# UtkarshMishra04/bioimitation-gym

Hardware: AMD Instinct MI355X
Metric: env steps/sec (whole node), MuscleWalkingImitation2D-v0 @ 4096 envs/GPU (higher is better)
Workload: dtype f64

## Files before the change

### bioimitation-gym_amd/csrc/bioim_step.hip

```cpp
#include <hip/hip_runtime.h>

#include <math.h>
#include <stdint.h>
#include <stdio.h>
#include <string.h>

#include <string>
#include <type_traits>
#include <memory>
#include <vector>

#include "bioim.h"
#include "bioim_device.h"
#include "topologies.h"

#define DEV __device__ __forceinline__
#define BIOIM_EPB 16
#define BIOIM_STRUCT_FLAGS (BIOIM_ENV_MUSCLE | BIOIM_ENV_HAS_TZ | BIOIM_ENV_REWARD_FEET | BIOIM_ENV_DONE_CROSS | BIOIM_ENV_PD)

#ifndef BIOIM_CHECK
#define BIOIM_CHECK 0
#endif
DEV size_t bioim_chk(size_t i, size_t n, int line) {
    if (i >= n) {
// ... 542 lines not shown
    static constexpr int U = ((MF + 3 * (NSLOT > 0 ? NSLOT : 1) + 1) / 2) * 2;
    static constexpr int LOC = U;
    static constexpr int SL = LOC + 24 * (NB + 1);
    static constexpr int TZ = MPL * T::G * T::MAXSPAN;
    static constexpr int TAUN = TZ + 1;
    static constexpr int TAU = U;
    static constexpr int CJ = TAU + TAUN;
    static constexpr int OBS = U;
    static constexpr int REP = OBS + OBSMAX;
    static constexpr int U1 = 24 * (NB + 1) + 6 * (ND + 1), U2 = TAUN + NS * CJN;
    static constexpr int U3 = OBSMAX + 6 * (T::NOS + 1);
    static constexpr int USZ = U1 > U2 ? (U1 > U3 ? U1 : U3) : (U2 > U3 ? U2 : U3);
    static constexpr int SIZE0 = ((U + USZ + 1) / 2) * 2;
    static constexpr int SIZE = (BIOIM_ENV_MOD >= 0 && T::PLANAR) ? SIZE0 + ((BIOIM_ENV_MOD - SIZE0 % 32) + 32) % 32 : SIZE0;
};

#ifndef BIOIM_REALIZE_CACHE
#define BIOIM_REALIZE_CACHE 1
#endif
#ifndef BIOIM_REALIZE_CACHE_SPATIAL
#define BIOIM_REALIZE_CACHE_SPATIAL 1
#endif
#ifndef BIOIM_REALIZE_CACHE_TORQUE
#define BIOIM_REALIZE_CACHE_TORQUE 1
#endif
#ifndef BIOIM_CACHE_PREFETCH_SPATIAL
#define BIOIM_CACHE_PREFETCH_SPATIAL 0
#endif
template <class T> struct CacheLay {
    static constexpr bool ON = BIOIM_REALIZE_CACHE &&
                               (T::NM > 0 ? (T::PLANAR || BIOIM_REALIZE_CACHE_SPATIAL) : BIOIM_REALIZE_CACHE_TORQUE);
    static constexpr bool PREFETCH = T::PLANAR || BIOIM_CACHE_PREFETCH_SPATIAL;
    static constexpr int ND = T::ND > 0 ? T::ND : 1, NP = ND * (ND + 1) / 2;
    static constexpr int SYS = NP + ND;
    static constexpr int MUS = SYS;
    static constexpr int H = MUS + 3 * T::NM;
    static constexpr int DIM = ON ? H + 1 : 0;
    static constexpr int PF = (SYS + T::G - 1) / T::G;
};

constexpr int PERT_SLOT = 5;

DEV void wave_sync() {
    __builtin_amdgcn_fence(__ATOMIC_RELEASE, "wavefront");
    __builtin_amdgcn_wave_barrier();
    __builtin_amdgcn_fence(__ATOMIC_ACQUIRE, "wavefront");
}
DEV void wave_sync_lanes() { wave_sync(); }

#ifdef BIOIM_STAMPS
#define STAMP(i)                                                                      \
    do {                                                                              \
        __builtin_amdgcn_sched_barrier(0);                                            \
        unsigned long long t_ = __builtin_amdgcn_s_memtime();                         \
        __builtin_amdgcn_s_waitcnt(0xC07F);                                           \
        if (blockIdx.x == 0 && threadIdx.x == 0) g_stamps[i] += t_ - stamp_prev;      \
        stamp_prev = t_;                                                              \
        __builtin_amdgcn_sched_barrier(0);                                            \
    } while (0)
#define STAMP_DECL unsigned long long stamp_prev = __builtin_amdgcn_s_memtime();
#else
#define STAMP(i) do {} while (0)
#define STAMP_DECL
#endif

template <int I> DEV constexpr int tri(int k, int l) { return k * (k + 1) / 2 + l; }

template <class T, typename Real>
DEV void publish_coords(const DModel<Real> &M, const SModel<T, Real> &SM, Real *lds, int lane, Real qd, Real ud) {
    using LY = Lay<T, Real>;
    if (lane < T::ND) {
        const int c = SM.dof_coord[lane];
        lds[LY::QF + c] = qd;
        lds[LY::UF + c] = ud;
    }
    if (lane == 0) {
        sfor<0, T::NC>([&](auto cI) {
            constexpr int c = decltype(cI)::value;
            if constexpr (T::coord_dof[c] < 0) { lds[LY::QF + c] = M.coord_default[c]; lds[LY::UF + c] = 0; }
        });
    }
}

template <class T, typename Real>
DEV void kin_local(const SModel<T, Real> &SM, Real *lds, int c) {
    using LY = Lay<T, Real>;
    using PL = Planar<T>;
    constexpr unsigned ZR = PL::ZR, ZW = PL::ZW, ZV = PL::ZV;
    constexpr unsigned USED = TopoInfo<T>::axes_used();
    const SBody<Real> &b = SM.body[c];
    Real RFM[9] = {1, 0, 0, 0, 1, 0, 0, 0, 1};
    Real wrel[3] = {0, 0, 0}, arel[3] = {0, 0, 0}, pFM[3] = {0, 0, 0}, pd[3] = {0, 0, 0}, pdd[3] = {0, 0, 0};
    Real col[6][3];
    int cd[6];
    sfor<0, 6>([&](auto aI) {
        constexpr int ax = decltype(aI)::value;
        cd[ax] = -1;
        if constexpr (((USED >> ax) & 1u) != 0) {
            int kind = -1, cc = -1, dof = -1, js = -1;
            int cb = c;
            if constexpr (!T::PLANAR) asm volatile("" : "+v"(cb));
            sfor<0, T::NB>([&](auto bI) {
                constexpr int bb = decltype(bI)::value;
                constexpr int k = T::axis_kind[bb * 6 + ax], co = T::axis_coord[bb * 6 + ax];
                constexpr int dc = co >= 0 ? T::coord_dof[co] : -1, jsl = TopoInfo<T>::jslot(bb, ax);
                kind = cb == bb ? k : kind;
                cc = cb == bb ? co : cc;
                dof = cb == bb ? dc : dof;
                js = cb == bb ? jsl : js;
            });
            const int cs = cc >= 0 ? cc : 0;
            Real qc = lds[LY::QF + cs], uc = lds[LY::UF + cs];
            qc = cc >= 0 ? qc : Real(0);
            uc = cc >= 0 ? uc : Real(0);
            constexpr unsigned KM = TopoInfo<T>::axis_kinds(ax);
            const Real fa = b.fa[ax], fb = b.fb[ax];
            Real f = 0, f1 = 0, f2 = 0;
            if constexpr ((KM & (1u << (BIOIM_FN_LINEAR + 1))) != 0) {
                if (kind == BIOIM_FN_LINEAR) { f = fa * qc + fb; f1 = fa; }
            }
            if constexpr ((KM & (1u << (BIOIM_FN_CONST + 1))) != 0) {
                if (kind == BIOIM_FN_CONST) f = fb;
            }
            if constexpr ((KM & (1u << (BIOIM_FN_SPLINE + 1))) != 0) {
                const int jj = js >= 0 ? js : 0;
                if constexpr (T::PLANAR) {
                    const bool sp = kind == BIOIM_FN_SPLINE;
                    const Real sf = lds[LY::MF + 3 * jj], sf1 = lds[LY::MF + 3 * jj + 1], sf2 = lds[LY::MF + 3 * jj + 2];
                    f = sp ? sf : f; f1 = sp ? sf1 : f1; f2 = sp ? sf2 : f2;
                } else if (kind == BIOIM_FN_SPLINE) {
                    f = lds[LY::MF + 3 * jj]; f1 = lds[LY::MF + 3 * jj + 1]; f2 = lds[LY::MF + 3 * jj + 2];
                }
            }
            cd[ax] = dof;
            Real a[3] = {b.axis[ax][0], b.axis[ax][1], b.axis[ax][2]};
            if constexpr (ax < 3) {
                PL::ang(a);
                Real ucol[3], cr[3];
                mv3m<ZR, ZW>(RFM, a, ucol);
                Real thd = f1 * uc;
                cross3m<ZW, ZW>(wrel, ucol, cr);
#pragma unroll
                for (int i = 0; i < 3; ++i) {
                    arel[i] += ucol[i] * (f2 * uc * uc) + cr[i] * thd;
                    wrel[i] += ucol[i] * thd;
                    col[ax][i] = ucol[i] * f1;
                }
                PL::ang(arel); PL::ang(wrel); PL::ang(col[ax]);
                Real Rk[9];
                if constexpr (T::PLANAR) {
                    Real sn, cn;
                    sincos_rt(f, sn, cn);
                    Rk[0] = cn; Rk[1] = -sn * a[2]; Rk[3] = sn * a[2]; Rk[4] = cn;
                    PL::rot(Rk);
                } else {
                    axis_rot(a, f, Rk);
                }
                mm3m<ZR, ZR>(RFM, Rk, RFM);
            } else {
#pragma unroll
                for (int i = 0; i < 3; ++i) {
                    pFM[i] += a[i] * f; pd[i] += a[i] * (f1 * uc); pdd[i] += a[i] * (f2 * uc * uc);
                    col[ax][i] = a[i] * f1;
                }
                PL::lin(pd); PL::lin(pdd); PL::lin(col[ax]);
            }
        }
    });
    Real Rpf[9], Rmb[9];
#pragma unroll
    for (int i = 0; i < 9; ++i) { Rpf[i] = b.R_pf[i]; Rmb[i] = b.R_mb[i]; }
    PL::rot(Rpf); PL::rot(Rmb);
    Real dF[3], T9[9], RPB[9], pm[3], pPB[3];
    mv3m<ZR, 0>(RFM, b.p_mb, dF);
    mm3m<ZR, ZR>(Rpf, RFM, T9);
    mm3m<ZR, ZR>(T9, Rmb, RPB);
#pragma unroll
    for (int i = 0; i < 3; ++i) pm[i] = pFM[i] + dF[i];
    mv3m<ZR, 0>(Rpf, pm, pPB);
    Real *lc = lds + LY::LOC + 24 * c;
#pragma unroll
    for (int i = 0; i < 9; ++i) lc[i] = RPB[i];
#pragma unroll
    for (int i = 0; i < 3; ++i) lc[9 + i] = pPB[i] + b.p_pf[i];
    Real t1[3], t2[3], t3[3], o[3];
    mv3m<ZR, ZW>(Rpf, wrel, o);
#pragma unroll
    for (int i = 0; i < 3; ++i) lc[12 + i] = o[i];
    cross3m<ZW, 0>(wrel, dF, t1);
#pragma unroll
    for (int i = 0; i < 3; ++i) t2[i] = pd[i] + t1[i];
    mv3m<ZR, ZV>(Rpf, t2, o);
#pragma unroll
    for (int i = 0; i < 3; ++i) lc[15 + i] = o[i];
    mv3m<ZR, ZW>(Rpf, arel, o);
#pragma unroll
    for (int i = 0; i < 3; ++i) lc[18 + i] = o[i];
    cross3m<ZW, 0>(arel, dF, t2);
    cross3m<ZW, ZV>(wrel, t1, t3);
#pragma unroll
    for (int i = 0; i < 3; ++i) t2[i] = pdd[i] + t2[i] + t3[i];
    mv3m<ZR, ZV>(Rpf, t2, o);
#pragma unroll
    for (int i = 0; i < 3; ++i) lc[21 + i] = o[i];
    Real pM[3];
    mv3m<ZR, 0>(Rpf, pFM, pM);
#pragma unroll
    for (int i = 0; i < 3; ++i) pM[i] += b.p_pf[i];
    sfor<0, 6>([&](auto aI) {
        constexpr int ax = decltype(aI)::value;
        if constexpr (((USED >> ax) & 1u) != 0) {
            if (T::PLANAR || cd[ax] >= 0) {
                Real *sl = lds + LY::SL + 6 * (cd[ax] >= 0 ? cd[ax] : LY::ND);
                Real v[3];
                if constexpr (ax < 3) {
                    mv3m<ZR, ZW>(Rpf, col[ax], v);
                    Real lin[3];
                    cross3m<0, ZW>(pM, v, lin);
#pragma unroll
                    for (int i = 0; i < 3; ++i) {
                        if (!((ZW >> i) & 1u)) sl[i] += v[i];
                        if (!((ZV >> i) & 1u)) sl[3 + i] += lin[i];
                    }
                } else {
                    mv3m<ZR, ZV>(Rpf, col[ax], v);
#pragma unroll
                    for (int i = 0; i < 3; ++i)
                        if (!((ZV >> i) & 1u)) sl[3 + i] += v[i];
                }
            }
        }
    });
}

template <typename Real> struct Frame {
    Real R[9], o[3], w[3], vO[3], al[3], aO[3];
};

template <class T, typename Real> DEV void compose(Frame<Real> &F, const Real *lc) {
    using PL = Planar<T>;
    constexpr unsigned ZR = PL::ZR, ZW = PL::ZW, ZV = PL::ZV;
    Real R[9], oB[3], w[3], wrg[3], vrel[3], vO[3], al[3], t[3], t2[3], t3[3];
    mm3m<ZR, ZR>(F.R, lc, R);
    mv3m<ZR, 0>(F.R, lc + 9, t);
#pragma unroll
    for (int i = 0; i < 3; ++i) oB[i] = F.o[i] + t[i];
    mv3m<ZR, ZW>(F.R, lc + 12, wrg);
#pragma unroll
    for (int i = 0; i < 3; ++i) w[i] = F.w[i] + wrg[i];
    mv3m<ZR, ZV>(F.R, lc + 15, vrel);
    cross3m<ZW, 0>(wrg, oB, t);
#pragma unroll
    for (int i = 0; i < 3; ++i) vO[i] = F.vO[i] + vrel[i] - t[i];
    mv3m<ZR, ZW>(F.R, lc + 18, t);
    cross3m<ZW, ZW>(F.w, wrg, t2);
#pragma unroll
    for (int i = 0; i < 3; ++i) al[i] = F.al[i] + t2[i] + t[i];
    Real vpt[3], aB[3], aa[3];
    cross3m<ZW, 0>(F.w, oB, t);
#pragma unroll
    for (int i = 0; i < 3; ++i) vpt[i] = F.vO[i] + t[i];
    cross3m<ZW, 0>(F.al, oB, t);
    cross3m<ZW, ZV>(F.w, vpt, t2);
    cross3m<ZW, ZV>(F.w, vrel, t3);
    mv3m<ZR, ZV>(F.R, lc + 21, aa);
#pragma unroll
    for (int i = 0; i < 3; ++i) aB[i] = F.aO[i] + t[i] + t2[i] + Real(2) * t3[i] + aa[i];
    Real vB[3];
    cross3m<ZW, 0>(w, oB, t);
#pragma unroll
    for (int i = 0; i < 3; ++i) vB[i] = vO[i] + t[i];
    cross3m<ZW, 0>(al, oB, t);
    cross3m<ZW, ZV>(w, vB, t2);
#pragma unroll
    for (int i = 0; i < 9; ++i) F.R[i] = R[i];
#pragma unroll
    for (int i = 0; i < 3; ++i) {
        F.aO[i] = aB[i] - t[i] - t2[i];
        F.o[i] = oB[i]; F.w[i] = w[i]; F.vO[i] = vO[i]; F.al[i] = al[i];
    }
    PL::rot(F.R); PL::ang(F.w); PL::lin(F.vO); PL::ang(F.al); PL::lin(F.aO);
}

#ifndef BIOIM_GROUND_ONCE
#define BIOIM_GROUND_ONCE 3
#endif
template <class T, typename Real> DEV constexpr bool ground_loc_free() {
    using LY = Lay<T, Real>;
    return LY::LOC + 24 * T::NB >= LY::TAU + LY::TAUN && LY::LOC + 24 * T::NB >= LY::CJ + LY::NS * LY::CJN;
}
template <class T, typename Real> DEV void kin_ground_loc(Real *lds) {
    Real *lc = lds + Lay<T, Real>::LOC + 24 * T::NB;
#pragma unroll
    for (int i = 0; i < 24; ++i) lc[i] = (i < 9 && (i % 4) == 0) ? Real(1) : Real(0);
}
template <class T, typename Real> DEV void kin_ground_const(Real *lds) {
    using LY = Lay<T, Real>;
    Real *kb = lds + LY::KB + 18 * T::NB, *ab = lds + LY::AL + 6 * T::NB;
#pragma unroll
    for (int i = 0; i < 18; ++i) kb[i] = (i < 9 && (i % 4) == 0) ? Real(1) : Real(0);
#pragma unroll
    for (int i = 0; i < 6; ++i) ab[i] = 0;
}
template <class T, typename Real, bool ONCE = false> DEV void kin_ground(Real *lds, Real x0) {
    if constexpr (!ONCE || !ground_loc_free<T, Real>()) kin_ground_loc<T, Real>(lds);
    if constexpr (!ONCE) kin_ground_const<T, Real>(lds);
    lds[Lay<T, Real>::KB + 18 * T::NB + 9] = -x0;
}

template <class T, typename Real>
DEV void kin_chain(const SModel<T, Real> &SM, Real *lds, int c, Real x0) {
    using LY = Lay<T, Real>;
    Frame<Real> F;
#pragma unroll
    for (int i = 0; i < 9; ++i) F.R[i] = (i % 4) == 0 ? Real(1) : Real(0);
#pragma unroll
    for (int i = 0; i < 3; ++i) { F.o[i] = i == 0 ? -x0 : Real(0); F.w[i] = 0; F.vO[i] = 0; F.al[i] = 0; F.aO[i] = 0; }
    sfor<0, TopoInfo<T>::depth()>([&](auto lI) {
        constexpr int lvl = decltype(lI)::value;
        const Real *src = lds + LY::LOC + 24 * SM.chain[c][lvl];
        Real lc[24];
#pragma unroll
        for (int i = 0; i < 24; ++i) lc[i] = src[i];
        Planar<T>::loc(lc);
        compose<T, Real>(F, lc);
    });
    Real *kb = lds + LY::KB + 18 * c, *ab = lds + LY::AL + 6 * c;
#pragma unroll
    for (int i = 0; i < 9; ++i) kb[i] = F.R[i];
#pragma unroll
    for (int i = 0; i < 3; ++i) {
        kb[9 + i] = F.o[i]; kb[12 + i] = F.w[i]; kb[15 + i] = F.vO[i];
        ab[i] = F.al[i]; ab[3 + i] = F.aO[i];
    }
}

template <bool BFK, class T, typename Real>
DEV void fn_slots(const SModel<T, Real> &SM, Real *lds, int lane) {
    using LY = Lay<T, Real>;
    if constexpr (LY::NSLOT > 0) {
        sfor<0, (LY::NSLOT + T::G - 1) / T::G>([&](auto pI) {
            const int f = lane + decltype(pI)::value * T::G;
            if (f < LY::NSLOT) {
                Real v, d1, d2;
                fn_eval_bf<BFK, T, Real>(SM, SM.mf_fn[f], lds[LY::QF + SM.mf_coord[f]], v, d1, d2);
                lds[LY::MF + 3 * f] = v;
                lds[LY::MF + 3 * f + 1] = d1;
                lds[LY::MF + 3 * f + 2] = d2;
            }
        });
        wave_sync();
    }
}

template <class T, typename Real>
DEV void kin_column(const SModel<T, Real> &SM, Real *lds, int d) {
    using LY = Lay<T, Real>;
    using PL = Planar<T>;
    constexpr unsigned ZR = PL::ZR, ZW = PL::ZW, ZV = PL::ZV;
    const Real *kp = lds + LY::KB + 18 * SM.body[SM.dof_cb[d]].pslot;
    const Real *sl = lds + LY::SL + 6 * d;
    Real K[12], sc[6];
#pragma unroll
    for (int i = 0; i < 12; ++i) K[i] = kp[i];
#pragma unroll
    for (int i = 0; i < 6; ++i) sc[i] = sl[i];
    PL::rot(K); PL::col(sc);
    Real Sa[3], Sl[3], t[3];
    mv3m<ZR, ZW>(K, sc, Sa);
    mv3m<ZR, ZV>(K, sc + 3, Sl);
    cross3m<ZW, 0>(Sa, K + 9, t);
    Real *S = lds + LY::S + 6 * d;
#pragma unroll
    for (int i = 0; i < 3; ++i) { S[i] = Sa[i]; S[3 + i] = Sl[i] - t[i]; }
}

template <class T, typename Real>
DEV void body_inertia(const SModel<T, Real> &SM, const DModel<Real> &M, Real *lds, int c) {
    using LY = Lay<T, Real>;
    using PL = Planar<T>;
    constexpr unsigned ZR = PL::ZR, ZW = PL::ZW, ZV = PL::ZV;
    const SBody<Real> &b = SM.body[c];
    const Real *kb = lds + LY::KB + 18 * c, *ab = lds + LY::AL + 6 * c;
    Real K[18], A[6];
#pragma unroll
    for (int i = 0; i < 18; ++i) K[i] = kb[i];
#pragma unroll
    for (int i = 0; i < 6; ++i) A[i] = ab[i];
    PL::frame(K); PL::acc(A);
    const Real *R = K, *o = K + 9, *w = K + 12, *vO = K + 15, *al = A, *aO = A + 3;
    Real cl[3], cG[3];
    mv3m<ZR, 0>(R, b.com, cl);
#pragma unroll
    for (int i = 0; i < 3; ++i) cG[i] = o[i] + cl[i];
    Real Ib[9] = {b.inertia[0], b.inertia[3], b.inertia[4], b.inertia[3], b.inertia[1],
                  b.inertia[5], b.inertia[4], b.inertia[5], b.inertia[2]};
    Real Tm[9], RT[9], IG[9];
#pragma unroll
    for (int i = 0; i < 3; ++i)
#pragma unroll
        for (int j = 0; j < 3; ++j) RT[3 * i + j] = R[3 * j + i];
    mm3m<ZR, 0>(R, Ib, Tm);
    mm3m<0, ZR>(Tm, RT, IG);
    Real m = b.mass, ccd = dot3(cG, cG);
    Real *ic = lds + LY::IC + 10 * c;
    ic[0] = m;
#pragma unroll
    for (int i = 0; i < 3; ++i) ic[1 + i] = m * cG[i];
    ic[4] = IG[0] + m * (ccd - cG[0] * cG[0]);
    ic[5] = IG[4] + m * (ccd - cG[1] * cG[1]);
    ic[6] = IG[8] + m * (ccd - cG[2] * cG[2]);
    ic[7] = IG[1] - m * cG[0] * cG[1];
    ic[8] = IG[2] - m * cG[0] * cG[2];
    ic[9] = IG[5] - m * cG[1] * cG[2];
    Real vc[3], ac[3], t[3], t2[3];
    cross3m<ZW, 0>(w, cG, t);
#pragma unroll
    for (int i = 0; i < 3; ++i) vc[i] = vO[i] + t[i];
    cross3m<ZW, 0>(al, cG, t);
    cross3m<ZW, ZV>(w, vc, t2);
#pragma unroll
    for (int i = 0; i < 3; ++i) ac[i] = aO[i] + t[i] + t2[i];
    Real f[3], Iw[3], Ia[3], n[3];
#pragma unroll
    for (int i = 0; i < 3; ++i) f[i] = m * (ac[i] - M.gravity[i]);
    mv3m<0, ZW>(IG, w, Iw);
    mv3m<0, ZW>(IG, al, Ia);
    cross3m<ZW, 0>(w, Iw, t);
#pragma unroll
    for (int i = 0; i < 3; ++i) n[i] = Ia[i] + t[i];
    cross3(cG, f, t);
    Real *wb = lds + LY::WB + 6 * c;
#pragma unroll
    for (int i = 0; i < 3; ++i) { wb[i] = n[i] + t[i]; wb[3 + i] = f[i]; }
}

template <unsigned ZB, typename Real> DEV void symvm(const Real *J, const Real *v, Real *o) {
    const int r0[3] = {0, 3, 4}, r1[3] = {3, 1, 5}, r2[3] = {4, 5, 2}, iv[3] = {0, 1, 2}, sg[3] = {1, 1, 1};
    Real x = sum_m<0, ZB, 3>(J, v, r0, iv, sg), y = sum_m<0, ZB, 3>(J, v, r1, iv, sg), z = sum_m<0, ZB, 3>(J, v, r2, iv, sg);
    o[0] = x; o[1] = y; o[2] = z;
}
template <typename Real> DEV void symv(const Real *J, const Real *v, Real *o) {
    Real x = J[0] * v[0] + J[3] * v[1] + J[4] * v[2];
    Real y = J[3] * v[0] + J[1] * v[1] + J[5] * v[2];
    Real z = J[4] * v[0] + J[5] * v[1] + J[2] * v[2];
    o[0] = x; o[1] = y; o[2] = z;
}

template <class T> struct DofTree {
    static constexpr int par(int d) {
        for (int e = d - 1; e >= 0; --e)
            if (T::dof_cb[e] == T::dof_cb[d]) return e;
        for (int b = T::parent[T::dof_cb[d]]; b >= 0; b = T::parent[b]) {
            int last = -1;
            for (int e = 0; e < T::ND; ++e)
                if (T::dof_cb[e] == b) last = e;
            if (last >= 0) return last;
        }
        return -1;
    }
    static constexpr bool anc(int k, int i) {
        for (int j = par(k); j >= 0; j = par(j))
            if (j == i) return true;
        return false;
    }
    static constexpr unsigned path_mask(int k) {
        unsigned m = 1u << k;
        for (int j = par(k); j >= 0; j = par(j)) m |= 1u << j;
        return m;
    }
    static constexpr bool root_common() {
// ... 414 lines not shown
                for (int i = 0; i < 3; ++i) P[i] += Rb[9 + i];
                mv3m<ZR, 0>(Rb, dloc, dP);
                Real e[3] = {0, 0, 0};
                if (have) {
                    Real sgm[3] = {P[0] - Pp[0], P[1] - Pp[1], P[2] - Pp[2]};
                    const Real l2 = dot3(sgm, sgm);
                    const Real inv = fast_rsqrt(l2), len = l2 * inv;
                    L += len;
#pragma unroll
                    for (int a = 0; a < 3; ++a) e[a] = sgm[a] * inv;
                    Real g[3] = {ep[0] - e[0], ep[1] - e[1], ep[2] - e[2]};
                    flush(g);
                }
#pragma unroll
                for (int a = 0; a < 3; ++a) { ep[a] = e[a]; Pp[a] = P[a]; dPp[a] = dP[a]; }
                maskp = pt.dofmask;
                mdofp = pt.mdof;
                have = true;
            }
        }
    });
    if (have) flush(ep);
}

template <class T, typename Real> struct Dyn {
    static constexpr int MPL = Lay<T, Real>::MPL;
    Real qdd;
    MState<Real> ms[MPL];
    Real act[MPL], lce[MPL];
    Real x0;
    bool ok;
};

template <typename Real> struct PertArgs {
    const double *x;
    const Real *y;
    int n, ob, env, N;
};

template <typename Real>
DEV Real pert_force(const PertArgs<Real> &P, double *sl, int k) {
    const double tc = sl[0] + (double)k * sl[1];
    if (!(tc >= sl[2] && tc < sl[3])) {
        int lo = -1, hi = P.n;
        while (hi - lo > 1) {
            const int mid = (lo + hi) >> 1;
            if (P.x[mid] <= tc) lo = mid; else hi = mid;
        }
        sl[2] = lo >= 0 ? P.x[lo] : -INFINITY;
        sl[3] = hi < P.n ? P.x[hi] : INFINITY;
        sl[4] = (double)GAT(P.y, (size_t)(lo >= 0 ? lo : 0) * P.N + P.env, (size_t)P.n * P.N);
    }
    return (Real)sl[4];
}

template <class T, typename Real> struct CacheIO {
    static constexpr int PF = CacheLay<T>::PF > 0 ? CacheLay<T>::PF : 1;
    static constexpr int PFA = CacheLay<T>::PREFETCH ? PF : 1, MPA = CacheLay<T>::PREFETCH ? Lay<T, Real>::MPL : 1;
    bool use = false, make = false;
    Real hc = 0;
    Real *base = nullptr;
    int env = 0, N = 0;
    DEV Real *row() const {
        int e = env;
        asm volatile("" : "+v"(e));
        return base + GIDX((size_t)e * CacheLay<T>::DIM, (size_t)N * CacheLay<T>::DIM);
    }
    Real sys[PFA];
    Real mus[MPA][3];
};

template <class T, bool IMP = true> struct BfSwitch {
    static constexpr bool BFK = (T::PLANAR || BIOIM_BF_SPATIAL) && (IMP || T::NM > 0);
    static constexpr bool BF3 = !T::PLANAR && (IMP || BIOIM_BF3_RK);
    static constexpr bool FN = BFK || (BF3 && (BIOIM_BF3 & 1)), PATH = BFK || (BF3 && (BIOIM_BF3 & 2));
    static constexpr bool CON = BFK || (BF3 && (BIOIM_BF3 & 4)), LIM = BFK || (BF3 && (BIOIM_BF3 & 8));
    static constexpr bool EQ = BFK || (BF3 && (BIOIM_BF3 & 16)), ROW = BFK || (BF3 && (BIOIM_BF3 & 32));
    static constexpr bool ME = BFK || (BF3 && (BIOIM_BF3 & 128));
};

template <class T, bool FUSED = false> struct TailSwitch {
    static constexpr int BIT = FUSED ? 4 : (T::PLANAR ? 1 : 2);
    static constexpr bool GROUND = (BIOIM_GROUND_ONCE & BIT) != 0;
};
template <class T, typename Real, bool PERT, bool BF_ROWS, bool IMP, bool CACHE = false, class TS = TailSwitch<T>>
DEV void dynamics(const DModel<Real> &M, const SModel<T, Real> &SM, Real qd, Real ud,
                  const Real (&act)[Lay<T, Real>::MPL], const Real (&lce)[Lay<T, Real>::MPL],
                  const Real (&control)[Lay<T, Real>::MPL], int lane, Real *lds, Real h, bool equilibrate,
                  const PertArgs<Real> &P, double *pslot, int pk, Dyn<T, Real> &D, const CacheIO<T, Real> &CI) {
    using LY = Lay<T, Real>;
    constexpr int ND = LY::ND, NP = LY::NP, NB = T::NB, G = T::G, MPL = LY::MPL;
    static_assert(!CACHE || (CacheLay<T>::ON && IMP && !PERT), "the realize cache: the default (semi-implicit, no push) step kernels");
    static_assert(NB < G && ND <= G, "lane NB writes the ground slot; one lane per dof");
    constexpr bool IMP_BF = IMP && (T::PLANAR || BIOIM_BF_SPATIAL || ((BIOIM_BF3 & 64) && !PERT));
    using SW = BfSwitch<T, IMP>;
    constexpr bool BFC = true;
    STAMP_DECL
    if (CACHE && CI.use) {
        using CL = CacheLay<T>;
        Real *const crow = CL::PREFETCH ? nullptr : CI.row();
#pragma unroll
        for (int i = 0; i < CacheIO<T, Real>::PF; ++i)
            if (lane + i * G < CL::SYS) {
                if constexpr (CL::PREFETCH) lds[LY::MP + lane + i * G] = CI.sys[i];
                else lds[LY::MP + lane + i * G] = GAT(crow, lane + i * G, CL::DIM);
            }
        if constexpr (T::NM > 0) {
#pragma unroll
            for (int j = 0; j < MPL; ++j) {
                const int m = mslot<T>(lane + j * G);
                if (m < T::NM) {
                    const SMuscle<Real> &mu = SM.mus[m];
                    const Real amin = mu.amin, one = 1, a_state = act[j];
                    const Real a = a_state < amin ? amin : (a_state > one ? one : a_state);
                    MState<Real> &s = D.ms[j];
                    Real cv[3];
#pragma unroll
                    for (int c = 0; c < 3; ++c) {
                        if constexpr (CL::PREFETCH) cv[c] = CI.mus[j][c];
                        else cv[c] = GAT(crow, CL::MUS + 3 * m + c, CL::DIM);
                    }
                    s.vN = cv[0];
                    s.vce = s.vN * mu.lv;
                    s.dvdl = cv[1];
                    s.clamped = cv[2] != Real(0);
                    s.dadt = act_rate<SW::ME>(mu, a, control[j]);
                }
            }
        } else {
            if (lane == 0) lds[LY::TAU + LY::TZ] = Real(0);
            sfor<0, MPL>([&](auto jI) {
                constexpr int j = decltype(jI)::value;
                const int m = mslot<T>(lane + j * G);
                if (m < T::NA) lds[LY::TAU + (lane + j * G) * T::MAXSPAN] = control[j] * SM.ca_opt[m];
            });
            wave_sync();
            if (lane < ND) {
                Real r = lds[LY::RHS + lane];
#pragma unroll
                for (int i = 0; i < T::MAXARM; ++i) r += lds[LY::TAU + SM.tau_src[lane][i]];
                lds[LY::RHS + lane] = r;
            }
        }
        wave_sync();
    } else {
    publish_coords<T, Real>(M, SM, lds, lane, qd, ud);
    if (lane < ND) {
#pragma unroll
        for (int i = 0; i < 6; ++i) lds[LY::SL + 6 * lane + i] = 0;
    }
    wave_sync();
    Real x0 = 0;
    if constexpr (T::TX >= 0) {
        if constexpr (T::coord_dof[T::TX] >= 0) x0 = M.float_origin ? lds[LY::QF + T::TX] : Real(0);
    }
    D.x0 = x0;

    fn_slots<SW::FN, T, Real>(SM, lds, lane);
    STAMP(15);

    if (lane < NB) kin_local<T, Real>(SM, lds, lane);
    if (lane == NB) kin_ground<T, Real, TS::GROUND>(lds, x0);
    wave_sync();
    STAMP(0);
    if (lane < NB) kin_chain<T, Real>(SM, lds, lane, x0);
    wave_sync();
    STAMP(1);
    if (lane < ND) kin_column<T, Real>(SM, lds, lane);
    if (lane < NB) {
        body_inertia<T, Real>(SM, M, lds, lane);
        if (PERT && lane == SM.os_cb[P.ob]) {
            const Real fpx = pert_force<Real>(P, pslot, pk);
            const Real *kb = lds + LY::KB + 18 * lane;
            Real p[3];
            mv3(kb, SM.os_p[P.ob], p);
            Real *wb = lds + LY::WB + 6 * lane;
            wb[1] -= (p[2] + kb[11]) * fpx;
            wb[2] += (p[1] + kb[10]) * fpx;
            wb[3] -= fpx;
        }
    }
    wave_sync();
    STAMP(2);

    {
        constexpr unsigned ICU = T::PLANAR ? 0x47u : 0x3FFu, WBU = T::PLANAR ? 0x1Cu : 0x3Fu;
        Real ic[10] = {0, 0, 0, 0, 0, 0, 0, 0, 0, 0}, wb[6] = {0, 0, 0, 0, 0, 0};
        if (lane < NB) {
            sfor<0, NB>([&](auto dI) {
                constexpr int d = decltype(dI)::value;
                const bool mine = (T::anc[d] >> lane) & 1u;
                if (T::PLANAR || mine) {
                    const Real on = !T::PLANAR || mine ? Real(1) : Real(0);
#pragma unroll
                    for (int i = 0; i < 10; ++i)
                        if ((ICU >> i) & 1u) ic[i] = fma(on, lds[LY::IC + 10 * d + i], ic[i]);
#pragma unroll
                    for (int i = 0; i < 6; ++i)
                        if ((WBU >> i) & 1u) wb[i] = fma(on, lds[LY::WB + 6 * d + i], wb[i]);
                }
            });
        }
        wave_sync();
        if (lane < NB) {
#pragma unroll
            for (int i = 0; i < 10; ++i)
                if ((ICU >> i) & 1u) lds[LY::IC + 10 * lane + i] = ic[i];
#pragma unroll
            for (int i = 0; i < 6; ++i)
                if ((WBU >> i) & 1u) lds[LY::WB + 6 * lane + i] = wb[i];
        }
    }
    STAMP(3);
    const Real hi = (CACHE && CI.make) ? CI.hc : h;
    constexpr bool MUSCLE_CONTACT = T::NM >= T::NS && T::NS > 0;
    ContactOut<Real> CO;
    if constexpr (T::NM > 0) {
        if (lane == 0) lds[LY::TAU + LY::TZ] = Real(0);
        sfor<0, MPL>([&](auto jI) {
            constexpr int j = decltype(jI)::value;
            const int m = mslot<T>(lane + j * G);
            if (m < T::NM) {
                const SMuscle<Real> &mu = SM.mus[m];
                Real L, dLs[T::MAXSPAN];
                muscle_path<SW::PATH, T, Real>(SM, mu, lds, L, dLs);
                STAMP(4);
                Real a_ = act[j], l_ = lce[j];
                if (equilibrate)
                    l_ = muscle_equilibrium<SW::EQ, T, Real>(SM, mu, a_, L);
                D.act[j] = a_;
                D.lce[j] = l_;
                if constexpr (j == 0 && MUSCLE_CONTACT) contact_compute<SW::CON, T, Real>(SM, lds, lane < T::NS ? lane : 0, hi, CO);
                muscle_eval<SW::ME, BFC, T, Real>(SM, mu, a_, l_, control[j], L, D.ms[j].vN, D.ms[j]);
                const Real nFt = -D.ms[j].Ft;
                Real *ts = lds + LY::TAU + (lane + j * G) * T::MAXSPAN;
#pragma unroll
                for (int k = 0; k < T::MAXSPAN; ++k) ts[k] = nFt * dLs[k];
            }
        });
    } else {
        if (lane == 0) lds[LY::TAU + LY::TZ] = Real(0);
        sfor<0, MPL>([&](auto jI) {
            constexpr int j = decltype(jI)::value;
            const int m = mslot<T>(lane + j * G);
            if (m < T::NA) lds[LY::TAU + (lane + j * G) * T::MAXSPAN] = control[j] * SM.ca_opt[m];
        });
    }
    STAMP(5);
    if constexpr (MUSCLE_CONTACT) {
        if (lane < T::NS) contact_store<T, Real>(lds, lane, CO);
    } else {
        if (lane < T::NS) contact_lane<SW::CON, T, Real>(SM, lds, lane, hi);
    }
    STAMP(6);
    if (lane < T::NL) {
        int cc = SM.lim_coord[lane];
        Real qv = lds[LY::QF + cc], qd = lds[LY::UF + cc];
        Real qup = SM.lim_qup[lane], qlo = SM.lim_qlow[lane], tr = SM.lim_trans[lane], itr = SM.lim_itrans[lane];
        Real up = smooth_step<SW::LIM>(Real(0), Real(1), qup, qup + tr, itr, qv);
        Real lo = smooth_step<SW::LIM>(Real(1), Real(0), qlo - tr, qlo, itr, qv);
        Real f = -SM.lim_kup[lane] * up * (qv - qup) + SM.lim_klow[lane] * lo * (qlo - qv) - SM.lim_damp[lane] * (up + lo) * qd;
        Real diag = 0, tadd = f;
        if (IMP_BF || (!IMP_BF && hi > 0)) {
            Real dup = smooth_step_d<SW::LIM>(Real(0), Real(1), qup, qup + tr, itr, qv);
            Real dlo = smooth_step_d<SW::LIM>(Real(1), Real(0), qlo - tr, qlo, itr, qv);
// ... 2193 lines not shown
            bk_tmv3(kb, kb + 12, wl);
            Il[0] = bd.inertia[0] * wl[0] + bd.inertia[3] * wl[1] + bd.inertia[4] * wl[2];
            Il[1] = bd.inertia[3] * wl[0] + bd.inertia[1] * wl[1] + bd.inertia[5] * wl[2];
            Il[2] = bd.inertia[4] * wl[0] + bd.inertia[5] * wl[1] + bd.inertia[2] * wl[2];
            mv3(kb, Il, Iw);
            Real *ic = lds + LY::IC + 10 * lane, *wb = lds + LY::WB + 6 * lane;
#pragma unroll
            for (int i = 0; i < 3; ++i) { ic[i] = cG[i]; ic[3 + i] = vc[i]; ic[6 + i] = ac[i]; wb[i] = Iw[i]; }
            ic[9] = Real(0.5) * (bd.mass * dot3(vc, vc) + dot3(wl, Il));
        }
        wave_sync();
        if (lane == 0) {
            Real mt = 0, ke = 0, cs[3] = {0, 0, 0}, vs[3] = {0, 0, 0}, as[3] = {0, 0, 0}, hs[3] = {0, 0, 0};
#pragma unroll 1
            for (int c = 0; c < NB; ++c) {
                const Real *ic = lds + LY::IC + 10 * c;
                const Real m = SM.body[c].mass;
#pragma unroll
                for (int i = 0; i < 3; ++i) { cs[i] += m * ic[i]; vs[i] += m * ic[3 + i]; as[i] += m * ic[6 + i]; }
                mt += m;
                ke += ic[9];
            }
            Real C0[3], V0[3];
#pragma unroll
            for (int i = 0; i < 3; ++i) { C0[i] = cs[i] / mt; V0[i] = vs[i] / mt; }
#pragma unroll 1
            for (int c = 0; c < NB; ++c) {
                const Real *ic = lds + LY::IC + 10 * c, *wb = lds + LY::WB + 6 * c;
                const Real m = SM.body[c].mass;
                Real r[3], dv[3], t[3];
#pragma unroll
                for (int i = 0; i < 3; ++i) { r[i] = ic[i] - C0[i]; dv[i] = ic[3 + i] - V0[i]; }
                cross3(r, dv, t);
#pragma unroll
                for (int i = 0; i < 3; ++i) hs[i] += wb[i] + m * t[i];
            }
            C0[0] += x0;
            if (a.system) {
                const size_t r9 = (size_t)idx * 9, rows = (size_t)a.n * 9;
#pragma unroll
                for (int i = 0; i < 3; ++i) {
                    GAT(a.system, r9 + i, rows) = C0[i]; GAT(a.system, r9 + 3 + i, rows) = V0[i];
                    GAT(a.system, r9 + 6 + i, rows) = as[i] / mt;
                }
            }
            if (a.momentum) {
                const size_t r6 = (size_t)idx * 6, rows = (size_t)a.n * 6;
#pragma unroll
                for (int i = 0; i < 3; ++i) { GAT(a.momentum, r6 + i, rows) = vs[i]; GAT(a.momentum, r6 + 3 + i, rows) = hs[i]; }
            }
            if (a.energy) {
                GAT(a.energy, (size_t)idx * 2, (size_t)a.n * 2) = ke;
                GAT(a.energy, (size_t)idx * 2 + 1, (size_t)a.n * 2) = -mt * dot3(M.gravity, C0);
            }
        }
    }
}

template <class T, typename Real, bool PERT, bool RK, bool REP, bool FUSED = false>
DEV void env_block(const LaunchArgs<T, Real> &a, int blk) {
    using LY = Lay<T, Real>;
    using TS = TailSwitch<T, FUSED>;
    constexpr int G = T::G, ND = LY::ND, NA = T::NA, NM = T::NM;
    constexpr int EPB = BIOIM_EPB;
    constexpr size_t SMB = smodel_bytes<T, Real>();
    extern __shared__ __attribute__((aligned(16))) unsigned char smem_raw[];
    const DModel<Real> *__restrict__ Mg = a.Mg;
    const DState<Real> &st = a.st;
    const int N = a.N, mode = REP ? 2 : a.mode;
    const bool osim = REP;
    const Real *__restrict__ actions = a.actions;
    Real *__restrict__ obs = a.obs;
#ifdef BIOIM_STAMPS
    const unsigned long long k_t0 = __builtin_amdgcn_s_memtime();
#endif
    {
        const uint4 *src = reinterpret_cast<const uint4 *>(a.Sg);
        uint4 *dst = reinterpret_cast<uint4 *>(smem_raw);
        for (int i = threadIdx.x; i < (int)(SMB / 16); i += BIOIM_EPB * G) dst[i] = src[i];
    }
    __syncthreads();
#ifdef BIOIM_STAMPS
    const unsigned long long k_t1 = __builtin_amdgcn_s_memtime();
    if (blockIdx.x == 0 && threadIdx.x == 0) g_stamps[11] += k_t1 - k_t0;
#endif
    const SModel<T, Real> &SM = *reinterpret_cast<const SModel<T, Real> *>(smem_raw);
    const DModel<Real> &M = *Mg;
    const int lane = threadIdx.x % G;
    const int slot = threadIdx.x / G;
    int gidx = blk * EPB + slot;
    Real *lds = reinterpret_cast<Real *>(smem_raw + SMB) + slot * LY::SIZE;
    int env;
    if (mode == 1 || osim) {
        if (gidx >= a.n_list) return;
        env = a.env_ids ? GAT(a.env_ids, gidx, a.n_list) : gidx;
        if (env < 0 || env >= N) return;
    } else {
        if (gidx >= N) return;
        env = gidx;
        if (a.active && !GAT(a.active, env, N) && !(RK && GAT(st.pend, env, (size_t)N) != 0)) return;
    }
    const int H = M.horizon;
    if constexpr (TS::GROUND) {
        if (lane == T::NB) {
            kin_ground_const<T, Real>(lds);
            if constexpr (ground_loc_free<T, Real>()) kin_ground_loc<T, Real>(lds);
        }
    }
    constexpr int MPL = LY::MPL;
    constexpr int CPL = (T::NC + G - 1) / G;
    Dyn<T, Real> D;
#pragma unroll
    for (int j = 0; j < MPL; ++j) D.ms[j].vN = 0;
#if BIOIM_FV_PRED
    Real vprev[MPL];
#pragma unroll
    for (int j = 0; j < MPL; ++j) vprev[j] = 0;
#endif
    Real qd = 0, ud = 0;
    if (lane < ND) { qd = GAT(st.q, (size_t)lane * N + env, (size_t)ND * N); ud = GAT(st.u, (size_t)lane * N + env, (size_t)ND * N); }
    double t = GAT(st.t, env, (size_t)N);
    int istep = GAT(st.istep, env, (size_t)N), has_last = REP ? 0 : GAT(st.has_last, env, (size_t)N),
        resets = REP ? 0 : GAT(st.resets, env, (size_t)N);
    Real old_px = REP ? Real(0) : GAT(st.old_px, env, (size_t)N);
    Real act[MPL], lce[MPL], control[MPL], curr[MPL], last[MPL], hist[MPL][BIOIM_MAX_HORIZON];
#pragma unroll
    for (int j = 0; j < MPL; ++j) {
        const int m = mslot<T>(lane + j * G);
        act[j] = 0; lce[j] = 0; control[j] = 0; curr[j] = 0; last[j] = 0;
        if (NM > 0 && m < NM) { act[j] = GAT(st.act, (size_t)m * N + env, (size_t)(NM > 0 ? NM : 1) * N); lce[j] = GAT(st.lce, (size_t)m * N + env, (size_t)(NM > 0 ? NM : 1) * N); }
#pragma unroll
        for (int hh = 0; hh < BIOIM_MAX_HORIZON; ++hh) hist[j][hh] = 0;
        if (m < NA) {
            if (!REP) last[j] = GAT(st.last, (size_t)m * N + env, (size_t)NA * N);
#pragma unroll
            for (int hh = 0; hh < BIOIM_MAX_HORIZON; ++hh)
                hist[j][hh] = hh < H ? GAT(st.hist, ((size_t)hh * NA + m) * N + env, (size_t)BIOIM_MAX_HORIZON * NA * N) : Real(0);
            if (osim) control[j] = GAT(st.ctl, (size_t)m * N + env, (size_t)NA * N);
        }
    }
    constexpr bool CACHE = CacheLay<T>::ON && !PERT && !RK && !REP;
    CacheIO<T, Real> CI;
    bool cache_valid = false;
    Real cache_h = 0;
    if constexpr (CACHE) {
        using CL = CacheLay<T>;
        CI.base = st.cache; CI.env = env; CI.N = N;
        Real *const crow = st.cache + GIDX((size_t)env * CL::DIM, (size_t)N * CL::DIM);
        cache_valid = mode == 0 && GAT(st.cache_ok, env, (size_t)N) != 0;
        cache_h = GAT(crow, CL::H, CL::DIM);
        if constexpr (CL::PREFETCH) {
#pragma unroll
            for (int i = 0; i < CacheIO<T, Real>::PF; ++i)
                CI.sys[i] = lane + i * G < CL::SYS ? GAT(crow, lane + i * G, CL::DIM) : Real(0);
#pragma unroll
            for (int j = 0; j < MPL; ++j) {
                const int m = mslot<T>(lane + j * G);
#pragma unroll
                for (int c = 0; c < 3; ++c) CI.mus[j][c] = m < NM ? GAT(crow, CL::MUS + 3 * m + c, CL::DIM) : Real(0);
            }
        }
    }
    int done = 0;
    Real rew = 0, inf[5] = {0, 0, 0, 0, 0};
    bool do_reset = (mode == 1);
    const bool budget = RK && !REP && a.rk_budget > 0;
    const bool resume = RK && mode == 0 && GAT(st.pend, env, (size_t)N) != 0;
// ... 2996 lines not shown
```

Before: 17.29 million.

## Restructure kinematics front end: register-accumulated columns, fused chain+inertia, ground compose

Adds a compile-time BIOIM_FRONTEND switch, enabled by default for planar models, that changes the kinematics front end in four ways. Body lanes accumulate their dof column contributions in registers and store each SL row once, so the zeroing pass and the read-modify-write adds to LDS go away. Linear and const joint functions use branch-free selects. Body inertia is computed straight from the register frame produced by kin_chain, which removes one wave_sync and the reload of the KB/AL entries. Level 0 composes with a specialized ground routine. The cost is more register pressure from the per-body accumulators and a static_assert requirement that each dof belongs to exactly one body.

```diff
diff --git a/bioimitation-gym_amd/csrc/bioim_step.hip b/bioimitation-gym_amd/csrc/bioim_step.hip
--- a/bioimitation-gym_amd/csrc/bioim_step.hip
+++ b/bioimitation-gym_amd/csrc/bioim_step.hip
@@ -648,7 +648,57 @@
     }
 }
 
-template <class T, typename Real>
+#ifndef BIOIM_FRONTEND
+#define BIOIM_FRONTEND 0x00000F
+#endif
+constexpr int FE_COLS = 1, FE_KINDS = 2, FE_INERTIA = 4, FE_LEVEL0 = 8;
+
+template <class T> struct BodyDofs {
+    static constexpr int dof_of(int b, int ax) {
+        const int co = T::axis_coord[b * 6 + ax];
+        return co >= 0 ? T::coord_dof[co] : -1;
+    }
+    static constexpr int slot(int b, int ax) {
+        const int d = dof_of(b, ax);
+        if (d < 0) return -1;
+        int n = 0;
+        for (int a = 0; a < ax; ++a) {
+            const int e = dof_of(b, a);
+            if (e < 0) continue;
+            bool seen = false;
+            for (int a2 = 0; a2 < a; ++a2) seen = seen || dof_of(b, a2) == e;
+            if (e == d) return n;
+            n += seen ? 0 : 1;
+        }
+        return n;
+    }
+    static constexpr int count(int b) {
+        int n = 0;
+        for (int ax = 0; ax < 6; ++ax) n = slot(b, ax) + 1 > n ? slot(b, ax) + 1 : n;
+        return n;
+    }
+    static constexpr int max_count() {
+        int n = 1;
+        for (int b = 0; b < T::NB; ++b) n = count(b) > n ? count(b) : n;
+        return n;
+    }
+    static constexpr int dof(int b, int k) {
+        for (int ax = 0; ax < 6; ++ax)
+            if (slot(b, ax) == k) return dof_of(b, ax);
+        return -1;
+    }
+    static constexpr bool covers_all() {
+        for (int d = 0; d < T::ND; ++d) {
+            int n = 0;
+            for (int b = 0; b < T::NB; ++b)
+                for (int k = 0; k < count(b); ++k) n += dof(b, k) == d ? 1 : 0;
+            if (n != 1) return false;
+        }
+        return true;
+    }
+};
+
+template <class T, typename Real, int FE = 0>
 DEV void kin_local(const SModel<T, Real> &SM, Real *lds, int c) {
     using LY = Lay<T, Real>;
     using PL = Planar<T>;
@@ -672,7 +722,8 @@
                 constexpr int dc = co >= 0 ? T::coord_dof[co] : -1, jsl = TopoInfo<T>::jslot(bb, ax);
                 kind = cb == bb ? k : kind;
                 cc = cb == bb ? co : cc;
-                dof = cb == bb ? dc : dof;
+                constexpr int dl = (FE & FE_COLS) ? BodyDofs<T>::slot(bb, ax) : dc;
+                dof = cb == bb ? dl : dof;
                 js = cb == bb ? jsl : js;
             });
             const int cs = cc >= 0 ? cc : 0;
@@ -682,11 +733,20 @@
             constexpr unsigned KM = TopoInfo<T>::axis_kinds(ax);
             const Real fa = b.fa[ax], fb = b.fb[ax];
             Real f = 0, f1 = 0, f2 = 0;
-            if constexpr ((KM & (1u << (BIOIM_FN_LINEAR + 1))) != 0) {
-                if (kind == BIOIM_FN_LINEAR) { f = fa * qc + fb; f1 = fa; }
-            }
-            if constexpr ((KM & (1u << (BIOIM_FN_CONST + 1))) != 0) {
-                if (kind == BIOIM_FN_CONST) f = fb;
+            if constexpr ((FE & FE_KINDS) && T::PLANAR) {
+                if constexpr ((KM & (1u << (BIOIM_FN_LINEAR + 1))) != 0) {
+                    const bool li = kind == BIOIM_FN_LINEAR;
+                    const Real lf = fa * qc + fb;
+                    f = li ? lf : f; f1 = li ? fa : f1;
+                }
+                if constexpr ((KM & (1u << (BIOIM_FN_CONST + 1))) != 0) f = kind == BIOIM_FN_CONST ? fb : f;
+            } else {
+                if constexpr ((KM & (1u << (BIOIM_FN_LINEAR + 1))) != 0) {
+                    if (kind == BIOIM_FN_LINEAR) { f = fa * qc + fb; f1 = fa; }
+                }
+                if constexpr ((KM & (1u << (BIOIM_FN_CONST + 1))) != 0) {
+                    if (kind == BIOIM_FN_CONST) f = fb;
+                }
             }
             if constexpr ((KM & (1u << (BIOIM_FN_SPLINE + 1))) != 0) {
                 const int jj = js >= 0 ? js : 0;
@@ -773,6 +833,59 @@
     mv3m<ZR, 0>(Rpf, pFM, pM);
 #pragma unroll
     for (int i = 0; i < 3; ++i) pM[i] += b.p_pf[i];
+    if constexpr ((FE & FE_COLS) != 0) {
+        constexpr int NLS = BodyDofs<T>::max_count();
+        static_assert(BodyDofs<T>::covers_all(), "FE_COLS: one body lane stores each dof's SL row");
+        Real acc[NLS][6];
+#pragma unroll
+        for (int k = 0; k < NLS; ++k)
+#pragma unroll
+            for (int i = 0; i < 6; ++i) acc[k][i] = 0;
+        sfor<0, 6>([&](auto aI) {
+            constexpr int ax = decltype(aI)::value;
+            if constexpr (((USED >> ax) & 1u) != 0) {
+                Real v[3], lin[3] = {0, 0, 0};
+                if constexpr (ax < 3) {
+                    mv3m<ZR, ZW>(Rpf, col[ax], v);
+                    cross3m<0, ZW>(pM, v, lin);
+                } else {
+                    mv3m<ZR, ZV>(Rpf, col[ax], v);
+                }
+#pragma unroll
+                for (int k = 0; k < NLS; ++k) {
+                    const bool on = cd[ax] == k;
+#pragma unroll
+                    for (int i = 0; i < 3; ++i) {
+                        if constexpr (ax < 3) {
+                            if (!((ZW >> i) & 1u)) acc[k][i] = on ? acc[k][i] + v[i] : acc[k][i];
+                            if (!((ZV >> i) & 1u)) acc[k][3 + i] = on ? acc[k][3 + i] + lin[i] : acc[k][3 + i];
+                        } else {
+                            if (!((ZV >> i) & 1u)) acc[k][3 + i] = on ? acc[k][3 + i] + v[i] : acc[k][3 + i];
+                        }
+                    }
+                }
+            }
+        });
+        int cb = c;
+        if constexpr (!T::PLANAR) asm volatile("" : "+v"(cb));
+        sfor<0, NLS>([&](auto kI) {
+            constexpr int k = decltype(kI)::value;
+            int dk = -1;
+            sfor<0, T::NB>([&](auto bI) {
+                constexpr int bb = decltype(bI)::value;
+                constexpr int dbk = BodyDofs<T>::dof(bb, k);
+                dk = cb == bb ? dbk : dk;
+            });
+            if (dk >= 0) {
+                Real *sl = lds + LY::SL + 6 * dk;
+#pragma unroll
+                for (int i = 0; i < 3; ++i) {
+                    if (!((ZW >> i) & 1u)) sl[i] = acc[k][i];
+                    if (!((ZV >> i) & 1u)) sl[3 + i] = acc[k][3 + i];
+                }
+            }
+        });
+    } else
     sfor<0, 6>([&](auto aI) {
         constexpr int ax = decltype(aI)::value;
         if constexpr (((USED >> ax) & 1u) != 0) {
@@ -848,6 +961,27 @@
     PL::rot(F.R); PL::ang(F.w); PL::lin(F.vO); PL::ang(F.al); PL::lin(F.aO);
 }
 
+template <class T, typename Real> DEV void compose_ground(Frame<Real> &F, const Real *lc, Real x0) {
+    using PL = Planar<T>;
+    constexpr unsigned ZW = PL::ZW, ZV = PL::ZV;
+    Real oB[3], vB[3], t[3], t2[3];
+#pragma unroll
+    for (int i = 0; i < 9; ++i) F.R[i] = lc[i];
+    oB[0] = lc[9] - x0; oB[1] = lc[10]; oB[2] = lc[11];
+    const Real *wrg = lc + 12, *vrel = lc + 15, *al = lc + 18, *aa = lc + 21;
+    cross3m<ZW, 0>(wrg, oB, t);
+#pragma unroll
+    for (int i = 0; i < 3; ++i) { F.o[i] = oB[i]; F.w[i] = wrg[i]; F.vO[i] = vrel[i] - t[i]; F.al[i] = al[i]; }
+    cross3m<ZW, 0>(F.w, oB, t);
+#pragma unroll
+    for (int i = 0; i < 3; ++i) vB[i] = F.vO[i] + t[i];
+    cross3m<ZW, 0>(al, oB, t);
+    cross3m<ZW, ZV>(F.w, vB, t2);
+#pragma unroll
+    for (int i = 0; i < 3; ++i) F.aO[i] = aa[i] - t[i] - t2[i];
+    PL::rot(F.R); PL::ang(F.w); PL::lin(F.vO); PL::ang(F.al); PL::lin(F.aO);
+}
+
 #ifndef BIOIM_GROUND_ONCE
 #define BIOIM_GROUND_ONCE 3
 #endif
@@ -874,10 +1008,9 @@
     lds[Lay<T, Real>::KB + 18 * T::NB + 9] = -x0;
 }
 
-template <class T, typename Real>
-DEV void kin_chain(const SModel<T, Real> &SM, Real *lds, int c, Real x0) {
+template <class T, typename Real, int FE = 0>
+DEV void kin_chain(const SModel<T, Real> &SM, Real *lds, int c, Real x0, Frame<Real> &F) {
     using LY = Lay<T, Real>;
-    Frame<Real> F;
 #pragma unroll
     for (int i = 0; i < 9; ++i) F.R[i] = (i % 4) == 0 ? Real(1) : Real(0);
 #pragma unroll
@@ -889,7 +1022,8 @@
 #pragma unroll
         for (int i = 0; i < 24; ++i) lc[i] = src[i];
         Planar<T>::loc(lc);
-        compose<T, Real>(F, lc);
+        if constexpr (lvl == 0 && (FE & FE_LEVEL0) != 0) compose_ground<T, Real>(F, lc, x0);
+        else compose<T, Real>(F, lc);
     });
     Real *kb = lds + LY::KB + 18 * c, *ab = lds + LY::AL + 6 * c;
 #pragma unroll
@@ -899,6 +1033,11 @@
         kb[9 + i] = F.o[i]; kb[12 + i] = F.w[i]; kb[15 + i] = F.vO[i];
         ab[i] = F.al[i]; ab[3 + i] = F.aO[i];
     }
+}
+template <class T, typename Real>
+DEV void kin_chain(const SModel<T, Real> &SM, Real *lds, int c, Real x0) {
+    Frame<Real> F;
+    kin_chain<T, Real>(SM, lds, c, x0, F);
 }
 
 template <bool BFK, class T, typename Real>
@@ -941,18 +1080,28 @@
     for (int i = 0; i < 3; ++i) { S[i] = Sa[i]; S[3 + i] = Sl[i] - t[i]; }
 }
 
-template <class T, typename Real>
-DEV void body_inertia(const SModel<T, Real> &SM, const DModel<Real> &M, Real *lds, int c) {
+template <class T, typename Real, bool FROM_FRAME = false>
+DEV void body_inertia(const SModel<T, Real> &SM, const DModel<Real> &M, Real *lds, int c, const Frame<Real> *F = nullptr) {
     using LY = Lay<T, Real>;
     using PL = Planar<T>;
     constexpr unsigned ZR = PL::ZR, ZW = PL::ZW, ZV = PL::ZV;
     const SBody<Real> &b = SM.body[c];
     const Real *kb = lds + LY::KB + 18 * c, *ab = lds + LY::AL + 6 * c;
     Real K[18], A[6];
-#pragma unroll
-    for (int i = 0; i < 18; ++i) K[i] = kb[i];
-#pragma unroll
-    for (int i = 0; i < 6; ++i) A[i] = ab[i];
+    if constexpr (FROM_FRAME) {
+#pragma unroll
+        for (int i = 0; i < 9; ++i) K[i] = F->R[i];
+#pragma unroll
+        for (int i = 0; i < 3; ++i) {
+            K[9 + i] = F->o[i]; K[12 + i] = F->w[i]; K[15 + i] = F->vO[i];
+            A[i] = F->al[i]; A[3 + i] = F->aO[i];
+        }
+    } else {
+#pragma unroll
+        for (int i = 0; i < 18; ++i) K[i] = kb[i];
+#pragma unroll
+        for (int i = 0; i < 6; ++i) A[i] = ab[i];
+    }
     PL::frame(K); PL::acc(A);
     const Real *R = K, *o = K + 9, *w = K + 12, *vO = K + 15, *al = A, *aO = A + 3;
     Real cl[3], cG[3];
@@ -1533,6 +1682,7 @@
 template <class T, bool FUSED = false> struct TailSwitch {
     static constexpr int BIT = FUSED ? 4 : (T::PLANAR ? 1 : 2);
     static constexpr bool GROUND = (BIOIM_GROUND_ONCE & BIT) != 0;
+    static constexpr int FE = (BIOIM_FRONTEND >> (FUSED ? 16 : (T::PLANAR ? 0 : 8))) & 0xFF;
 };
 template <class T, typename Real, bool PERT, bool BF_ROWS, bool IMP, bool CACHE = false, class TS = TailSwitch<T>>
 DEV void dynamics(const DModel<Real> &M, const SModel<T, Real> &SM, Real qd, Real ud,
@@ -1595,10 +1745,13 @@
         }
         wave_sync();
     } else {
+    constexpr int FE = TS::FE;
     publish_coords<T, Real>(M, SM, lds, lane, qd, ud);
-    if (lane < ND) {
-#pragma unroll
-        for (int i = 0; i < 6; ++i) lds[LY::SL + 6 * lane + i] = 0;
+    if constexpr (!(FE & FE_COLS)) {
+        if (lane < ND) {
+#pragma unroll
+            for (int i = 0; i < 6; ++i) lds[LY::SL + 6 * lane + i] = 0;
+        }
     }
     wave_sync();
     Real x0 = 0;
@@ -1610,16 +1763,11 @@
     fn_slots<SW::FN, T, Real>(SM, lds, lane);
     STAMP(15);
 
-    if (lane < NB) kin_local<T, Real>(SM, lds, lane);
+    if (lane < NB) kin_local<T, Real, FE>(SM, lds, lane);
     if (lane == NB) kin_ground<T, Real, TS::GROUND>(lds, x0);
     wave_sync();
     STAMP(0);
-    if (lane < NB) kin_chain<T, Real>(SM, lds, lane, x0);
-    wave_sync();
-    STAMP(1);
-    if (lane < ND) kin_column<T, Real>(SM, lds, lane);
-    if (lane < NB) {
-        body_inertia<T, Real>(SM, M, lds, lane);
+    auto push = [&]() {
         if (PERT && lane == SM.os_cb[P.ob]) {
             const Real fpx = pert_force<Real>(P, pslot, pk);
             const Real *kb = lds + LY::KB + 18 * lane;
@@ -1630,8 +1778,31 @@
             wb[2] += (p[1] + kb[10]) * fpx;
             wb[3] -= fpx;
         }
-    }
-    wave_sync();
+    };
+    if constexpr ((FE & FE_INERTIA) != 0) {
+        if (lane < NB) {
+            Frame<Real> F;
+            kin_chain<T, Real, FE>(SM, lds, lane, x0, F);
+            body_inertia<T, Real, true>(SM, M, lds, lane, &F);
+            push();
+        }
+        wave_sync();
+        STAMP(1);
+        if (lane < ND) kin_column<T, Real>(SM, lds, lane);
+    } else {
+        if (lane < NB) {
+            Frame<Real> F;
+            kin_chain<T, Real, FE>(SM, lds, lane, x0, F);
+        }
+        wave_sync();
+        STAMP(1);
+        if (lane < ND) kin_column<T, Real>(SM, lds, lane);
+        if (lane < NB) {
+            body_inertia<T, Real>(SM, M, lds, lane);
+            push();
+        }
+        wave_sync();
+    }
     STAMP(2);
 
     {
@@ -3991,7 +4162,7 @@
     __syncthreads();
 #ifdef BIOIM_STAMPS
     const unsigned long long k_t1 = __builtin_amdgcn_s_memtime();
-    if (blockIdx.x == 0 && threadIdx.x == 0) g_stamps[11] += k_t1 - k_t0;
+    if (blockIdx.x == 0 && threadIdx.x == 0) { g_stamps[11] += k_t1 - k_t0; g_stamps[26] = 1 + TS::FE; }
 #endif
     const SModel<T, Real> &SM = *reinterpret_cast<const SModel<T, Real> *>(smem_raw);
     const DModel<Real> &M = *Mg;
```

Result: faster. 17.77 million, median of 6 (+2.8%).
